# t-0hmura/pdb2reaction

Hardware: AMD Instinct MI355X
Metric: path_opt_string_iterations_per_s (higher is better)
Workload: dtype bf16x3-split

## Files before the change

pdb2reaction_amd/csrc/umx_api.hip:

```cpp
#include "umx_engine.h"
#include "umx_launch.h"
#include "umx_workspace.h"
#include "umx_periodic.h"
#include "umx_virial.h"
#include "umx_plan.h"
#include "umx_weights.h"
#include "umx_experts.h"

#define NOT_MERGED "expert-form weights are loaded but not merged: call umx_set_expert_coefficients first (then umx_set_system)"

namespace {
int energy_forces_dev_impl(umx_engine* eng, int n_images, const PosPtr d_pos, double* d_energy, float* d_forces, double* d_virial, void* hip_stream) {
  if (!eng) return UMX_ERR_ARG;
  if (eng->need_merge()) return fail(eng, UMX_ERR_ARG, "umx_energy_forces: " NOT_MERGED);
  if (!eng->have_system) return fail(eng, UMX_ERR_ARG, "umx_energy_forces: bind a system first (umx_set_system)");
  if (n_images <= 0 || !(d_pos.f || d_pos.d) || !d_energy) return fail(eng, UMX_ERR_ARG, "umx_energy_forces: bad arguments");
  if (d_virial && !d_forces) return fail(eng, UMX_ERR_ARG, "umx_energy_forces_virial: the virial comes out of the reverse pass: ask for the forces too");
  if (eng->gp_plan) return fail(eng, UMX_ERR_ARG, "umx_energy_forces: a graph-parallel evaluation is in progress (finish it with umx_gp_step)");
  CHK(periodic_check_images(eng, n_images, "umx_energy_forces"));
  HIPCHK(eng, hipSetDevice(eng->dev));
  return energy_forces_on(eng, static_cast<hipStream_t>(hip_stream), n_images, d_pos, d_energy, d_forces, d_virial);
}

template <typename P>
// ... 149 lines not shown
#ifndef UMX_SRC_DIGEST
#define UMX_SRC_DIGEST "unknown"
#endif
const char* umx_build_digest(void) { return UMX_SRC_DIGEST; }

const char* umx_last_error(const umx_engine* eng) { return eng ? eng->err.c_str() : g_create_err.c_str(); }

int umx_create(umx_engine** out, int device_ordinal) {
  if (!out) { g_create_err = "umx_create: null out pointer"; return UMX_ERR_ARG; }
  *out = nullptr;
  int n = 0;
  if (hipGetDeviceCount(&n) != hipSuccess || n <= 0) { g_create_err = "umx_create: no HIP device visible"; return UMX_ERR_NO_DEVICE; }
  if (device_ordinal < 0 || device_ordinal >= n) { g_create_err = "umx_create: device ordinal out of range"; return UMX_ERR_ARG; }
  hipDeviceProp_t prop;
  if (hipGetDeviceProperties(&prop, device_ordinal) != hipSuccess) { g_create_err = "umx_create: hipGetDeviceProperties failed"; return UMX_ERR_HIP; }
  if (std::string(prop.gcnArchName).rfind("gfx950", 0) != 0) {
    g_create_err = std::string("umx_create: device is ") + prop.gcnArchName + ", this library is built for gfx950 only";
    return UMX_ERR_NO_DEVICE;
  }
  umx_engine* e = new umx_engine();
  e->dev = device_ordinal;
  if (const char* ev = std::getenv("UMX_STREAMS")) e->n_lanes = std::atoi(ev) >= 2 ? 2 : (std::atoi(ev) == 1 ? 1 : 0);
  if (const char* ev = std::getenv("UMX_LANES_AUTO_EDGES")) e->lanes_auto_edges = std::max(0L, std::atol(ev));
  if (const char* ev = std::getenv("UMX_FORCE_PARTS")) e->force_parts = std::max(0, std::min(16, std::atoi(ev)));
  if (const char* ev = std::getenv("UMX_RECOMPUTE")) e->recompute = std::max(0, std::min(2, std::atoi(ev)));
  if (const char* ev = std::getenv("UMX_WS_GB")) e->ws_cap_default = (size_t)std::max(0L, std::atol(ev)) << 30;
  if (const char* ev = std::getenv("UMX_WS_EAGER")) e->ws_eager = std::atoi(ev) != 0;
  if (const char* ev = std::getenv("UMX_WS_SOFT_EDGES")) e->ws_soft_edges = std::max(1L, std::atol(ev));
  if (const char* ev = std::getenv("UMX_NODE_F64")) e->node_f64_on = std::atoi(ev) != 0;
  if (const char* ev = std::getenv("UMX_GRID_F64")) e->grid_f64 = std::atoi(ev) != 0;
  if (const char* ev = std::getenv("UMX_ALT_ROWS")) e->odd_sign = std::atoi(ev) != 0 ? -1.0f : 1.0f;
  if (const char* ev = std::getenv("UMX_LOW_SEP")) e->low_sep = std::atoi(ev);
  if (const char* ev = std::getenv("UMX_GEMM_HALF")) e->gemm_half = std::atoi(ev);
  if (const char* ev = std::getenv("UMX_ALIGN_PLANES")) e->align = std::atoi(ev);
  int prio_lo = 0, prio_hi = 0;
  if (hipSetDevice(device_ordinal) != hipSuccess || hipDeviceGetStreamPriorityRange(&prio_lo, &prio_hi) != hipSuccess ||
      hipStreamCreateWithFlags(&e->stream, hipStreamNonBlocking) != hipSuccess ||
      hipStreamCreateWithPriority(&e->stream2, hipStreamNonBlocking, prio_hi) != hipSuccess ||
      hipEventCreateWithFlags(&e->ev_fork, hipEventDisableTiming) != hipSuccess || hipEventCreateWithFlags(&e->ev_join, hipEventDisableTiming) != hipSuccess ||
      hipEventCreateWithFlags(&e->ev_tok[0], hipEventDisableTiming) != hipSuccess || hipEventCreateWithFlags(&e->ev_tok[1], hipEventDisableTiming) != hipSuccess ||
      hipEventCreateWithFlags(&e->ev_done, hipEventDisableTiming) != hipSuccess || hipMalloc(&e->d_flags, 4 * sizeof(int)) != hipSuccess ||
      hipMemset(e->d_flags, 0, 4 * sizeof(int)) != hipSuccess) {
    g_create_err = "umx_create: hipSetDevice/hipStreamCreate failed";
    delete e;
    return UMX_ERR_HIP;
  }
  *out = e;
  return UMX_OK;
}


int umx_destroy(umx_engine* eng) {
  if (!eng) return UMX_OK;
  gp_clear(eng);
  (void)hipSetDevice(eng->dev);
  (void)hipStreamSynchronize(eng->stream);
  for (auto& r : eng->prof) { (void)hipEventDestroy(r.a); (void)hipEventDestroy(r.b); }
  void* ptrs[] = {eng->d_w, eng->d_dw, eng->d_bw, eng->d_gmu, eng->d_z, eng->d_sysemb, eng->arena, eng->d_deg_all, eng->d_cand_all, eng->d_img_edges, eng->d_io_pos, eng->d_io_e, eng->d_io_f, eng->d_flags, eng->d_dtab, eng->d_part_deg, eng->d_part_f, eng->d_ex, eng->d_mjobs, eng->d_pjobs, eng->d_mx, eng->d_cells, eng->d_shifts_pk, eng->d_wrap, eng->d_wrap64, eng->d_lats, eng->d_io_pos64, eng->d_vir_part, eng->d_vir_wp, eng->d_io_w, eng->d_pin_src, eng->d_pin_dst, eng->d_pin_tix, eng->d_pin_wrap, eng->d_pin_deg, eng->d_pin_img, eng->d_pin_shifts};
  for (void* p : ptrs) if (p) (void)hipFree(p);
  (void)hipStreamSynchronize(eng->stream2);
  (void)hipEventDestroy(eng->ev_fork); (void)hipEventDestroy(eng->ev_join);
  (void)hipEventDestroy(eng->ev_tok[0]); (void)hipEventDestroy(eng->ev_tok[1]);
  if (eng->ev_done) (void)hipEventDestroy(eng->ev_done);
  if (eng->ev_m0) { (void)hipEventDestroy(eng->ev_m0); (void)hipEventDestroy(eng->ev_m1); }
  (void)hipStreamDestroy(eng->stream2);
  (void)hipStreamDestroy(eng->stream);
// ... 383 lines not shown
  if (!eng) return UMX_ERR_ARG;
  if (out) std::memset(out, 0, sizeof(*out));
  HIPCHK(eng, hipSetDevice(eng->dev));
  HIPCHK(eng, hipStreamSynchronize(eng->stream));
  if (eng->prof_used) HIPCHK(eng, hipEventSynchronize(eng->prof[eng->prof_used - 1].b));
  FILE* dump = nullptr;
  if (const char* dp = std::getenv("UMX_PROFILE_DUMP")) dump = std::fopen(dp, "a");
  for (size_t i = 0; i < eng->prof_used; ++i) {
    float t = 0.f;
    HIPCHK(eng, hipEventElapsedTime(&t, eng->prof[i].a, eng->prof[i].b));
    const ProfRec& r = eng->prof[i];
    if (out) {
      const int fam = r.prec > 0 ? 0 : (r.prec < 0 ? 2 : 1);
      out->ms[fam] += t; out->launches[fam] += 1; out->alg_flops[fam] += r.flops;
      out->mfma_flops[fam] += r.flops * (r.prec == 3 ? 6.0 : r.prec == 2 ? 3.0 : r.prec == 24 ? 4.0 : r.prec == 23 ? 3.0 : r.prec == 28 ? 6.0 : 1.0);
    }
    if (dump) std::fprintf(dump, "%d,%d,%d,%d,%d,%d,%d,%.6f,%.6e\n", r.M, r.N, r.K, r.amode, r.cplx, r.prec, r.gz, t, r.flops);
  }
  if (dump) std::fclose(dump);
  if (reset) eng->prof_used = 0;
  return UMX_OK;
}

int umx_debug_keep(umx_engine* eng, int on) {
  if (!eng) return UMX_ERR_ARG;
  eng->dbg_on = on != 0;
  if (!on) { eng->dbg.clear(); eng->gemm_log.clear(); }
  return UMX_OK;
}

int umx_debug_fetch(umx_engine* eng, const char* name, void* host_buf, size_t capacity, size_t* nbytes_out) {
  if (!eng || !name) return UMX_ERR_ARG;
  const std::string nm(name);
  if (nm == "gemm:table" || nm == "gemm:launches") {
    const std::string text = nm == "gemm:table" ? pl_table_text() : eng->gemm_log;
    if (nbytes_out) *nbytes_out = text.size();
    if (host_buf) {
      if (capacity < text.size()) return fail(eng, UMX_ERR_ARG, "umx_debug_fetch: buffer too small");
      std::memcpy(host_buf, text.data(), text.size());
    }
    return UMX_OK;
  }
  if (nm.rfind("weights:", 0) == 0 || nm.rfind("experts:", 0) == 0) {
    if (!eng->have_weights) return fail(eng, UMX_ERR_ARG, "umx_debug_fetch: load weights first");
    HIPCHK(eng, hipSetDevice(eng->dev));
    HIPCHK(eng, hipStreamSynchronize(eng->stream));
    const void* dptr = nullptr; size_t nb = 0;
    std::string table; float ms = 0.f;
    if (nm == "weights:w") { dptr = eng->d_w; nb = eng->n_w * sizeof(float); }
    else if (nm == "weights:dw") { dptr = eng->d_dw; nb = eng->n_dw * sizeof(float); }
    else if (nm == "weights:bw") { dptr = eng->d_bw; nb = eng->n_bw * sizeof(unsigned short); }
    else if (nm == "weights:table") {
      for (const auto& kv : eng->wt) table += kv.first + " " + std::to_string(kv.second.off) + " " + std::to_string(kv.second.count) + "\n";
      nb = table.size();
    } else if (nm == "experts:kernel_ms") {
      if (!eng->experts_merged) return fail(eng, UMX_ERR_ARG, "umx_debug_fetch: no expert merge has run");
      HIPCHK(eng, hipEventElapsedTime(&ms, eng->ev_m0, eng->ev_m1));
      nb = sizeof(float);
    } else return fail(eng, UMX_ERR_ARG, std::string("umx_debug_fetch: no buffer named ") + name);
    if (nbytes_out) *nbytes_out = nb;
    if (host_buf) {
      if (capacity < nb) return fail(eng, UMX_ERR_ARG, "umx_debug_fetch: buffer too small");
      if (dptr) HIPCHK(eng, hipMemcpy(host_buf, dptr, nb, hipMemcpyDeviceToHost));
      else if (nm == "weights:table") std::memcpy(host_buf, table.data(), nb);
      else std::memcpy(host_buf, &ms, nb);
    }
    return UMX_OK;
  }
// ... 72 lines not shown
```

pdb2reaction_amd/csrc/umx_engine.h:

```cpp
#pragma once
#include <hip/hip_runtime.h>
#include <algorithm>
#include <cmath>
#include <cstdio>
#include <cstdlib>
#include <chrono>
#include <cstring>
#include <functional>
#include <initializer_list>
#include <map>
#include <memory>
#include <set>
#include <string>
#include <type_traits>
#include <vector>

#include "../../include/umx.h"
#include "umx_common.h"
#include "umx_gemm.h"
#include "umx_gemm_pl.h"
#include "umx_gemm_q.h"
#include "umx_kernels.h"
#include "umx_edge.h"
#include "umx_graph.h"
// ... 109 lines not shown

struct Seg { bool matrix; std::function<int()> fn; float* sync_buf = nullptr; size_t sync_count = 0; };
struct Plan {
  std::vector<Seg> segs;
  void stream(std::function<int()> f) { segs.push_back({false, std::move(f)}); }
  void matrix(std::function<int()> f) { segs.push_back({true, std::move(f)}); }
  void sync(float* buf, size_t count) { Seg sg{false, nullptr}; sg.sync_buf = buf; sg.sync_count = count; segs.push_back(std::move(sg)); }
  int run_to_sync(size_t& at, const Seg** stop) {
    *stop = nullptr;
    while (at < segs.size()) {
      Seg& sg = segs[at++];
      if (sg.sync_buf) { *stop = &sg; return UMX_OK; }
      const int st = sg.fn();
      if (st != UMX_OK) return st;
    }
    return UMX_OK;
  }
};

}

struct umx_engine {
  int dev = 0;
  hipStream_t stream = nullptr;
  hipEvent_t ev_done = nullptr;
  bool ran_on_caller = false;
  int* d_flags = nullptr;
  hipStream_t stream2 = nullptr;
  hipEvent_t ev_fork = nullptr, ev_join = nullptr;
  hipEvent_t ev_tok[2] = {nullptr, nullptr};
  Precision prec;
  std::string precision;
  int low_sep = 3;
  int gemm_half = 5;
  int align = 2;
  float odd_sign = -1.0f;
  bool node_ctx = false;
  bool node_f64_on = true;
  int n_lanes = 0;
  long lanes_auto_edges = 0;
  int stream_cap = 512;
  bool throttle = false;
  bool gp = false; long gp_lo = 0, gp_hi = 0;
  std::unique_ptr<Plan> gp_plan;
  std::unique_ptr<WS> gp_ws;
  size_t gp_at = 0;
  hipStream_t gp_stream = nullptr;
  std::string err;
  bool have_weights = false;
  float* d_w = nullptr;
  float* d_dw = nullptr;
  double* d_dtab = nullptr;
  unsigned short* d_bw = nullptr;
  std::map<const float*, PlaneCopy> planes;
  std::map<std::string, Tensor> wt;
  std::vector<float> h_w;
  size_t n_w = 0, n_dw = 0, n_bw = 0;
  int n_experts = 0;
  bool experts_merged = false;
  float* d_ex = nullptr;
  MergeJob* d_mjobs = nullptr; PackJob* d_pjobs = nullptr; unsigned* d_mx = nullptr;
  int n_mjobs = 0, n_pjobs = 0, merge_blocks = 0, pack_blocks = 0;
  std::vector<const float*> f16_keys;
  hipEvent_t ev_m0 = nullptr, ev_m1 = nullptr;
  bool need_merge() const { return n_experts > 0 && !experts_merged; }
  RadialW rdeg{};
// ... 156 lines not shown
```

pdb2reaction_amd/csrc/umx_gemm_pl.h:

```cpp
#pragma once
#include "umx_gemm.h"

namespace umx {

typedef float f32x4 __attribute__((ext_vector_type(4)));

struct GemmPL {
  const unsigned short* Apl; long lda; int offA0, offA1;
  const unsigned short* Bpl; long ldb; int bHalf;
  float* Cp; long ldc; int offC, offCi;
  const float* bias;
  float conj;
  int M, N, K;
  float cscale;
  float odd_sign;
};

template <int N> __device__ __forceinline__ void wait_vmcnt() {
  asm volatile("s_waitcnt vmcnt(%0)" ::"n"(N) : "memory");
}

template <int P> __device__ __forceinline__ int pl_perm(int s, int r) {
  return P == 2 ? (s ^ ((r >> 1) & 7)) : ((s & ~3) | ((s & 3) ^ ((r >> 2) & 3)));
}

template <int JA, int JB, int TA_B, int WSTR, long TAG>
__device__ __forceinline__ void pl_issue(const GemmPL& p, unsigned char* sbase, const long (&a_off)[JA], const long (&b_off)[JB], long kofs_a, long kofs, int piece) {
#pragma unroll
  for (int j = 0; j < JA; ++j)
    __builtin_amdgcn_global_load_lds(p.Apl + a_off[j] + kofs_a, (__attribute__((address_space(3))) void*)(sbase + piece + j * WSTR), 16, 0, 0);
#pragma unroll
  for (int j = 0; j < JB; ++j)
    __builtin_amdgcn_global_load_lds(p.Bpl + b_off[j] + kofs, (__attribute__((address_space(3))) void*)(sbase + TA_B + piece + j * WSTR), 16, 0, 0);
}

template <int E> struct PlMfma;
template <> struct PlMfma<32> {
  static constexpr int NR = 16, KSTEPS = 2;
  typedef f32x16 Acc;
  static __device__ __forceinline__ int row(int lane) { return lane & 31; }
  static __device__ __forceinline__ int kc(int lane) { return lane >> 5; }
  static __device__ __forceinline__ Acc mfma(const bf16x8_t& a, const bf16x8_t& b, const Acc& c) { return __builtin_amdgcn_mfma_f32_32x32x16_bf16(a, b, c, 0, 0, 0); }
};
template <> struct PlMfma<16> {
  static constexpr int NR = 4, KSTEPS = 1;
  typedef f32x4 Acc;
  static __device__ __forceinline__ int row(int lane) { return lane & 15; }
  static __device__ __forceinline__ int kc(int lane) { return lane >> 4; }
// ... 171 lines not shown
```

pdb2reaction_amd/csrc/umx_gemm_q.h:

```cpp
#pragma once
#include <type_traits>
#include "umx_gemm_pl.h"

namespace umx {

template <int P> __device__ __forceinline__ int q_row_off(int row) { return (row >> 2) * (128 * P) + (row & 3) * (32 * P); }
template <int P> __device__ __forceinline__ int q_swz(int g) { return P == 3 ? ((g >> 2) & 1) : ((g >> 1) & 3); }
typedef _Float16 f16x8_t __attribute__((ext_vector_type(8)));

template <int JA, int JBF, int BHALF_ROUND, int A_BYTES, long TAG, int RND = 8192, class BO = long>
__device__ __forceinline__ void q3_issue(const unsigned char* A, const unsigned char* B, unsigned char* sbase, const BO (&a_off)[JA],
                                         const BO (&b_off)[JBF + BHALF_ROUND], long kofs_a, long kofs_b, int piece, bool b_tail) {
  BO ao[JA];
#pragma unroll
  for (int j = 0; j < JA; ++j) {
    ao[j] = a_off[j];
    if constexpr (sizeof(BO) == 4) asm("" : "+v"(ao[j]));
  }
#pragma unroll
  for (int j = 0; j < JA; ++j)
    __builtin_amdgcn_global_load_lds((A + kofs_a) + ao[j], (__attribute__((address_space(3))) void*)(sbase + piece + j * RND), 16, 0, 0);
  BO bo[JBF + BHALF_ROUND];
#pragma unroll
  for (int j = 0; j < JBF + BHALF_ROUND; ++j) {
    bo[j] = b_off[j];
    if constexpr (sizeof(BO) == 4) asm("" : "+v"(bo[j]));
  }
#pragma unroll
  for (int j = 0; j < JBF; ++j)
    __builtin_amdgcn_global_load_lds((B + kofs_b) + bo[j], (__attribute__((address_space(3))) void*)(sbase + A_BYTES + piece + j * RND), 16, 0, 0);
  if constexpr (BHALF_ROUND != 0)
    if (b_tail)
      __builtin_amdgcn_global_load_lds((B + kofs_b) + bo[JBF], (__attribute__((address_space(3))) void*)(sbase + A_BYTES + piece + JBF * RND), 16, 0, 0);
}

__host__ __device__ constexpr bool q_use_product(int PA, int PB, int NPROD, int qa, int qb) {
  if (PA == 3 && PB == 3) return qa + qb < 3;
  if (PA == 2 && PB == 3) return NPROD == 5 ? (qa + qb < 3) : (qa + qb < 2 || (qa == 0 && qb == 2));
  return NPROD == 4 ? true : (qa + qb < 2);
}

template <int CPLX, int WIDE, int P = 3, int S = 2, int F16 = 0, int NPROD = (P == 3 ? 6 : 3), int PB = P, int AF = 0, int LS = 0, int AL = 0, int MW = 4>
__global__ __launch_bounds__(MW * 128, MW == 4 ? 1 : 2) void umx_gemm_q_kernel(const GemmPL p) {
  static_assert(!AL || AF, "AL: the float32-A kernels");
  static_assert(!LS || (P == 3 && PB == 3 && !F16 && NPROD == 6), "LS: the six-product bf16 form");
  static_assert(LS != 2 || !WIDE, "LS = 2 (second accumulator set): 256 x 128 tiles only");
  static_assert(MW == 4 || MW == 2, "waves along M: 4 (256-row tiles) or 2 (half-height tiles, two workgroups per CU)");
  static_assert(!AF || (P == 3 && PB == 3 && F16 == 0), "AF: the six-product bf16 form with A as float32");
  static_assert((P == 3 && PB == 3 && NPROD == 6) || (P == 2 && PB == 2 && (NPROD == 3 || NPROD == 4)) || (P == 2 && PB == 3 && (NPROD == 4 || NPROD == 5)), "plane products");
  constexpr int NT = MW * 128, RND = NT * 16;
  constexpr int BM = 64 * MW, BN = WIDE ? 256 : 128;
  constexpr int BMR = CPLX ? BM / 2 : BM, BNC = CPLX ? BN / 2 : BN;
  constexpr int BLK = AF ? 256 : 128 * P, CPB = AF ? 16 : 8 * P;
  constexpr int BLKB = 128 * PB, CPBB = 8 * PB;
  constexpr int A_BYTES = AF ? BM * 64 : BM * 32 * P, B_BYTES = BN * 32 * PB, STAGE = A_BYTES + B_BYTES;
  constexpr int TNW = WIDE ? 4 : 2;
  constexpr int JA = A_BYTES / RND;
  constexpr int JBF = B_BYTES / RND, BHR = (B_BYTES % RND) ? 1 : 0;
  static_assert(S * STAGE * (MW == 4 ? 1 : 2) <= 160 * 1024 && A_BYTES % RND == 0 && (B_BYTES % RND == 0 || B_BYTES % RND == RND / 2), "tile geometry");
  static_assert((P == 2 || P == 3) && (PB == 2 || PB == 3), "two or three planes");
  static_assert(S >= 2 && S <= 4, "ring depth");
  __shared__ __attribute__((aligned(1024))) unsigned char ring[S * STAGE];
  const int tid = threadIdx.x, lane = tid & 63, wave = tid >> 6;
  const int wm = wave >> 1, wn = wave & 1;
  const int l31 = lane & 31, h = lane >> 5;

  int mt, nt;
  if (!xcd_tile<BMR, BNC>(p.M, p.N, mt, nt)) return;

  const unsigned char* Ab = reinterpret_cast<const unsigned char*>(p.Apl);
  const unsigned char* Bb = reinterpret_cast<const unsigned char*>(p.Bpl);
  const long a_blocks = p.lda / (16 * P);
  const long b_blocks = p.K / 16;
  const long gA = ((long)p.M + 3) / 4;
  const int gN = p.N / 4;
  typedef typename std::conditional<MW == 4, long, unsigned int>::type BOff;
  BOff a_off[JA], b_off[JBF + BHR];
// ... 32 lines not shown
        for (int r = 0; r < 16; ++r) low[i][j][r] = 0.f;
  }
#pragma unroll
  for (int j = 0; j < TNW; ++j) {
    float b0 = 0.f;
    if (!CPLX) {
      const int col = nt * BN + wn * (32 * TNW) + j * 32 + l31;
      b0 = (p.bias && col < p.N) ? p.bias[col] / cs : 0.f;
    }
    const float b1 = p.odd_sign < 0.f ? -b0 : b0;
#pragma unroll
    for (int i = 0; i < 2; ++i)
#pragma unroll
      for (int r = 0; r < 16; ++r) acc[i][j][r] = (r & 1) ? b1 : b0;
  }

  int a_ad[2][P], b_ad[TNW][PB];
#pragma unroll
  for (int t = 0; t < 2; ++t) {
    const int row = frag_row0<CPLX, 2, 32, BMR>(wm, t) + l31;
#pragma unroll
    for (int q = 0; q < P; ++q)
      a_ad[t][q] = AF ? ((row >> 2) * 256 + (row & 3) * 64 + ((((h * 2 + (q & 1)) ^ ((row >> 2) & 3))) * 16))
                      : (q_row_off<P>(row) + ((q * 2 + h) ^ q_swz<P>(row >> 2)) * 16);
  }
#pragma unroll
  for (int t = 0; t < TNW; ++t) {
    const int row = frag_row0<CPLX, TNW, 32, BNC>(wn, t) + l31;
#pragma unroll
    for (int q = 0; q < PB; ++q) b_ad[t][q] = A_BYTES + q_row_off<PB>(row) + ((q * 2 + h) ^ q_swz<PB>(row >> 2)) * 16;
  }

  const int nk = p.K / 16;
  constexpr long TAG = kernel_tag<CPLX, WIDE, P, S, F16, NPROD, PB, AF, LS, AL, MW>();
  constexpr int GI = JA + JBF;
#pragma unroll
  for (int t = 0; t < S - 1; ++t)
    if (t < nk) q3_issue<JA, JBF, BHR, A_BYTES, TAG, RND, BOff>(Ab + a_tile, Bb, ring + t * STAGE, a_off, b_off, (long)t * BLK, (long)t * BLKB, piece, b_tail);
  int st_cur = 0, st_nxt = S - 1;
  for (int kt = 0; kt < nk; ++kt) {
    if (S == 2 || kt + S - 2 >= nk) wait_vmcnt<0>();
    else if (BHR != 0 && b_tail) wait_vmcnt<(S - 2) * (GI + 1)>();
    else wait_vmcnt<(S - 2) * GI>();
    __builtin_amdgcn_s_barrier();
    if (kt + S - 1 < nk) q3_issue<JA, JBF, BHR, A_BYTES, TAG, RND, BOff>(Ab + a_tile, Bb, ring + st_nxt * STAGE, a_off, b_off, (long)(kt + S - 1) * BLK, (long)(kt + S - 1) * BLKB, piece, b_tail);
    const unsigned char* sb = ring + st_cur * STAGE;
    st_cur = st_cur + 1 == S ? 0 : st_cur + 1;
    st_nxt = st_nxt + 1 == S ? 0 : st_nxt + 1;
    bf16x8_t a[2][P], b[TNW][PB];
    if constexpr (AF) {
#pragma unroll
      for (int t = 0; t < 2; ++t)
        qf_split<AL>(*reinterpret_cast<const f32x4q_t*>(sb + a_ad[t][0]), *reinterpret_cast<const f32x4q_t*>(sb + a_ad[t][1]), a[t]);
    } else {
#pragma unroll
      for (int q = 0; q < P; ++q)
#pragma unroll
        for (int t = 0; t < 2; ++t) a[t][q] = *reinterpret_cast<const bf16x8_t*>(sb + a_ad[t][q]);
    }
#pragma unroll
    for (int q = 0; q < PB; ++q)
#pragma unroll
      for (int t = 0; t < TNW; ++t) b[t][q] = *reinterpret_cast<const bf16x8_t*>(sb + b_ad[t][q]);
    if constexpr (LS == 1) {
#pragma unroll
      for (int i = 0; i < 2; ++i)
#pragma unroll
// ... 16 lines not shown
          lo = __builtin_amdgcn_mfma_f32_32x32x16_f16(__builtin_bit_cast(f16x8_t, a[i][0]), __builtin_bit_cast(f16x8_t, b[j][2]), lo, 0, 0, 0);
          lo = __builtin_amdgcn_mfma_f32_32x32x16_f16(__builtin_bit_cast(f16x8_t, a[i][0]), __builtin_bit_cast(f16x8_t, b[j][1]), lo, 0, 0, 0);
          lo = __builtin_amdgcn_mfma_f32_32x32x16_f16(__builtin_bit_cast(f16x8_t, a[i][1]), __builtin_bit_cast(f16x8_t, b[j][0]), lo, 0, 0, 0);
          acc[i][j] = __builtin_amdgcn_mfma_f32_32x32x16_f16(__builtin_bit_cast(f16x8_t, a[i][0]), __builtin_bit_cast(f16x8_t, b[j][0]), acc[i][j], 0, 0, 0);
          fold_low(acc[i][j], lo);
        }
    } else
#pragma unroll
    for (int ord = P + PB - 2; ord >= 0; --ord)
#pragma unroll
      for (int qa = 0; qa < P; ++qa) {
        const int qb = ord - qa;
        if (qb < 0 || qb >= PB || !q_use_product(P, PB, NPROD, qa, qb)) continue;
#pragma unroll
        for (int i = 0; i < 2; ++i)
#pragma unroll
          for (int j = 0; j < TNW; ++j) {
            if constexpr (F16) acc[i][j] = __builtin_amdgcn_mfma_f32_32x32x16_f16(__builtin_bit_cast(f16x8_t, a[i][qa]), __builtin_bit_cast(f16x8_t, b[j][qb]), acc[i][j], 0, 0, 0);
            else if constexpr (LS == 2) {
              if (qa + qb == 2) low[i][j] = __builtin_amdgcn_mfma_f32_32x32x16_bf16(a[i][qa], b[j][qb], low[i][j], 0, 0, 0);
              else acc[i][j] = __builtin_amdgcn_mfma_f32_32x32x16_bf16(a[i][qa], b[j][qb], acc[i][j], 0, 0, 0);
            } else acc[i][j] = __builtin_amdgcn_mfma_f32_32x32x16_bf16(a[i][qa], b[j][qb], acc[i][j], 0, 0, 0);
          }
      }
  }
  if constexpr (LS == 2) {
#pragma unroll
    for (int i = 0; i < 2; ++i)
#pragma unroll
      for (int j = 0; j < TNW; ++j) fold_low(acc[i][j], low[i][j]);
  }

  const bool full = ((long)mt * BMR + BMR <= p.M) && (nt * BNC + BNC <= p.N);
  if (CPLX) {
#pragma unroll
    for (int cg = 0; cg < TNW / 2; ++cg) {
      const int chan = nt * BNC + wn * (16 * TNW) + cg * 32 + l31;
      const long e0 = (long)mt * BMR + wm * 32 + 4 * h;
      float* c = p.Cp + e0 * p.ldc + chan;
      if (full) {
#pragma unroll
        for (int r = 0; r < 16; ++r) {
          float* cr = c + (long)cd_row<16>(r) * p.ldc;
          cr[p.offC] = ((r & 1) ? cso : cs) * (acc[0][cg][r] - p.conj * acc[1][TNW / 2 + cg][r]);
          cr[p.offCi] = ((r & 1) ? cso : cs) * (acc[1][cg][r] + p.conj * acc[0][TNW / 2 + cg][r]);
        }
      } else if (chan < p.N) {
#pragma unroll
        for (int r = 0; r < 16; ++r) {
          const int dr = cd_row<16>(r);
          if (e0 + dr < p.M) {
            float* cr = c + (long)dr * p.ldc;
            cr[p.offC] = ((r & 1) ? cso : cs) * (acc[0][cg][r] - p.conj * acc[1][TNW / 2 + cg][r]);
            cr[p.offCi] = ((r & 1) ? cso : cs) * (acc[1][cg][r] + p.conj * acc[0][TNW / 2 + cg][r]);
          }
        }
      }
    }
  } else {
#pragma unroll
    for (int i = 0; i < 2; ++i)
#pragma unroll
      for (int j = 0; j < TNW; ++j) {
        const int col = nt * BN + wn * (32 * TNW) + j * 32 + l31;
        const long row0 = (long)mt * BM + wm * 64 + i * 32 + 4 * h;
        float* c = p.Cp + row0 * p.ldc + p.offC + col;
        if (full) {
// ... 15 lines not shown
```

pdb2reaction_amd/csrc/umx_launch.h:

```cpp
#pragma once

namespace {

int prof_open(umx_engine* eng, ProfRec** out, double flops, int prec, long M, int N, int K, int amode = 0, int cplx = 0, int gz = 1) {
  *out = nullptr;
  if (!eng->prof_on) return UMX_OK;
  if (eng->prof_used == eng->prof.size()) {
    ProfRec r; HIPCHK(eng, hipEventCreate(&r.a)); HIPCHK(eng, hipEventCreate(&r.b)); r.flops = 0; eng->prof.push_back(r);
  }
  ProfRec* pr = &eng->prof[eng->prof_used++];
  pr->flops = flops; pr->M = (int)M; pr->N = N; pr->K = K; pr->amode = amode; pr->cplx = cplx; pr->gz = gz; pr->prec = prec;
  HIPCHK(eng, hipEventRecord(pr->a, eng->stream));
  *out = pr;
  return UMX_OK;
}
int prof_close(umx_engine* eng, ProfRec* pr) {
  if (pr) HIPCHK(eng, hipEventRecord(pr->b, eng->stream));
  return UMX_OK;
}
inline unsigned vgrid(const umx_engine* eng, unsigned blocks) {
  return (eng->throttle && eng->stream_cap > 0 && blocks > (unsigned)eng->stream_cap) ? (unsigned)eng->stream_cap : blocks;
}

inline void launch_scan(hipStream_t s, const int* deg, long n, int* row_ptr, int* stats) {
// ... 60 lines not shown
  return launch_gemm(eng, p, R ? A_MODUL : A_PLAIN, 1);
}

int so3_linear(umx_engine* eng, const float* A, const float* Wl, const float* bias, float* Cp, long nn, const float* resid) {
  GemmP p = gp_zero();
  p.A = A; p.lda = ROW; p.offA0 = 0; p.B = Wl; p.ldb = C; p.bias = bias; p.Cp = Cp; p.ldc = ROW; p.offC = 0;
  p.M = (int)nn; p.N = C; p.K = C; p.zA = C; p.zC = C; p.resid = resid; p.ldres = ROW; p.offRes = 0; p.zRes = C; p.zBl = (long)C * C;
  NodeCtx node(eng);
  return launch_gemm(eng, p, A_PLAIN, 0, S);
}

enum PlFamily { Q_F16, Q_BF16, PL3_ROWS, PL3, PL2_WIDE, PL2_M16, PL2_M32 };

struct PlKey {
  PlFamily fam = Q_F16; bool cplx = false, wide = false, ls = false, al = false, half = false;
  bool operator==(const PlKey& o) const { return fam == o.fam && cplx == o.cplx && wide == o.wide && ls == o.ls && al == o.al && half == o.half; }
};
struct PlKernel { PlKey key; void (*fn)(const GemmPL); };

#define UMX_Q(cplx, wide, ls, al, half) \
  {{Q_BF16, cplx != 0, wide != 0, ls != 0, al != 0, half != 0}, umx_gemm_q_kernel<cplx, wide, 3, 2, 0, 6, 3, 1, (ls ? (wide ? 1 : 2) : 0), al, (half ? 2 : 4)>}
#define UMX_Q4(cplx, wide, ls) UMX_Q(cplx, wide, ls, 0, 0), UMX_Q(cplx, wide, ls, 1, 0), UMX_Q(cplx, wide, ls, 0, 1), UMX_Q(cplx, wide, ls, 1, 1)
const PlKernel pl_kernels[] = {
    {{Q_F16, false, false}, umx_gemm_q_kernel<0, 0, 2, 2, 1, 4, 3>}, {{Q_F16, true, false}, umx_gemm_q_kernel<1, 0, 2, 2, 1, 4, 3>},
    {{Q_F16, false, true}, umx_gemm_q_kernel<0, 1, 2, 2, 1, 4, 3>},  {{Q_F16, true, true}, umx_gemm_q_kernel<1, 1, 2, 2, 1, 4, 3>},
    UMX_Q4(0, 0, 0), UMX_Q4(0, 0, 1), UMX_Q4(0, 1, 0), UMX_Q4(0, 1, 1),
    UMX_Q4(1, 0, 0), UMX_Q4(1, 1, 0), UMX_Q4(1, 1, 1),
    {{PL3_ROWS}, umx_gemm_pl_kernel<16, 0, 3, 2, 4, 2, 2, 2, 1>},
    {{PL3}, umx_gemm_pl_kernel<32, 0, 3, 2, 4, 2, 2, 2>},
    {{PL2_WIDE, false, true}, umx_gemm_pl_kernel<16, 0, 2, 2, 4, 2, 2, 4>}, {{PL2_WIDE, true, true}, umx_gemm_pl_kernel<16, 1, 2, 2, 4, 2, 2, 4>},
    {{PL2_M16, false}, umx_gemm_pl_kernel<16, 0, 2, 3, 4, 2, 2, 2>},        {{PL2_M16, true}, umx_gemm_pl_kernel<16, 1, 2, 3, 4, 2, 2, 2>},
    {{PL2_M32, false}, umx_gemm_pl_kernel<32, 0, 2, 3, 4, 2, 2, 2>},
};
#undef UMX_Q
#undef UMX_Q4
std::string pl_key_text(const PlKey& k) {
  static const char* const fam[] = {"Q_F16", "Q_BF16", "PL3_ROWS", "PL3", "PL2_WIDE", "PL2_M16", "PL2_M32"};
  return std::string(fam[k.fam]) + " " + std::to_string(k.cplx) + " " + std::to_string(k.wide) + " " + std::to_string(k.ls) + " " + std::to_string(k.al) + " " +
         std::to_string(k.half);
}
std::string pl_table_text() {
  std::string t;
  for (const PlKernel& e : pl_kernels) t += pl_key_text(e.key) + "\n";
  return t;
}

struct PlChoice { PlKey key; unsigned blocks = 0; long lda = 0, ldb = 0; int prec = 0; const char* err = nullptr; };
PlChoice choose_pl(const Precision& pm, Pass pass, bool w_quad, int cplx, long M, int N, int K, int a_cols, bool a_f32rows, int low_sep, int align, int half) {
  PlChoice c;
  c.key.cplx = cplx != 0;
  const bool fwd = pass == FWD;
  const int P = fwd ? 3 : pm.rev_planes;
  c.prec = (fwd && pm.fwd_fmt == 1) ? 24 : P;
  c.lda = (long)a_cols * P; c.ldb = (long)K * P;
  const int bmr = cplx ? 128 : 256;
  const long nM = (M + bmr - 1) / bmr;
  const bool fills = nM * (N / (cplx ? 128 : 256)) >= 256;
  c.key.ls = fwd && pm.fwd_fmt == 3 && (low_sep == 2 || (low_sep == 3 && !cplx) || (low_sep == 1 && !cplx && K == RH));
  c.key.wide = N % (cplx ? 128 : 256) == 0 && (fills || c.key.ls);
  int bnc = c.key.wide ? (cplx ? 128 : 256) : (cplx ? 64 : 128);
  if (fwd && pm.fwd_fmt == 1) {
    c.key.fam = Q_F16; c.lda = (long)a_cols * 2; c.ldb = (long)K * 3;
  } else if (fwd || (P == 3 && w_quad)) {
    c.key.fam = Q_BF16; c.lda = (long)a_cols * 3; c.ldb = (long)K * 3;
    c.key.al = fwd && (align == 1 || (align == 2 && !cplx));
  } else if (P == 3) {
    if (cplx || N > 128) { c.err = "gemm_pl: three-plane PL products are instantiated for the plain N <= 128 (radial fc3^T) products only"; return c; }
    c.key.fam = a_f32rows ? PL3_ROWS : PL3;
    if (a_f32rows) c.lda = (long)a_cols * 2;
  } else if (c.key.wide) {
    c.key.fam = PL2_WIDE;
  } else {
    c.key.fam = (cplx || K >= 512) ? PL2_M16 : PL2_M32;
  }
  c.key.half = c.key.fam == Q_BF16 && (half == 3 || (half == 4 && cplx) || (half == 5 && !c.key.ls && K >= 256) ||
                               (fwd && c.key.ls && (half == 2 || (half == 1 && !c.key.wide))));
  const long nMf = c.key.half ? (M + bmr / 2 - 1) / (bmr / 2) : nM;
  c.blocks = (unsigned)(((nMf + 7) / 8) * 8 * ((N + bnc - 1) / bnc));
  return c;
}

int gemm_pl(umx_engine* eng, int cplx, Pass pass, const unsigned short* Apl, int a_cols, int offA0, int offA1, const float* Wkey, int bHalf,
            const float* bias, float* Cp, long ldc, int offC, int offCi, long M, int N, int K, float conj, bool a_f32rows = false) {
  if (M <= 0) return UMX_OK;
  auto it = eng->planes.find(Wkey);
  if (it == eng->planes.end()) return fail(eng, UMX_ERR_ARG, "gemm_pl: weight has no PL copy");
  if (K % 32 != 0) return fail(eng, UMX_ERR_ARG, "gemm_pl: K not a multiple of 32");
  const PlaneCopy& w = it->second;
  const PlChoice c = choose_pl(eng->prec, pass, w.quad, cplx, M, N, K, a_cols, a_f32rows, eng->low_sep, eng->align, eng->gemm_half);
  if (c.err) return fail(eng, UMX_ERR_ARG, c.err);
  const PlKernel* k = nullptr;
  for (const PlKernel& e : pl_kernels)
    if (e.key == c.key) { k = &e; break; }
  if (!k) return fail(eng, UMX_ERR_ARG, "gemm_pl: variant not instantiated");
  GemmPL q;
  std::memset(&q, 0, sizeof(q));
  q.Apl = Apl; q.lda = c.lda; q.offA0 = offA0; q.offA1 = offA1; q.Bpl = w.ptr; q.ldb = c.ldb; q.bHalf = bHalf;
  q.Cp = Cp; q.ldc = ldc; q.offC = offC; q.offCi = offCi; q.bias = bias; q.conj = conj; q.M = (int)M; q.N = N; q.K = K;
  q.odd_sign = eng->odd_sign;
  if (c.key.fam == Q_F16) q.cscale = 1.0f / (QF16_SCALE * w.scale);
  ProfRec* pr;
  CHK(prof_open(eng, &pr, cplx ? 8.0 * M * (double)N * K : 2.0 * M * (double)N * K, c.prec, M, N, K, 9, cplx));
  hipLaunchKernelGGL(k->fn, dim3(c.blocks), dim3(c.key.half ? 256 : 512), 0, eng->stream, q);
  HIPCHK(eng, hipGetLastError());
  if (eng->dbg_on)
    eng->gemm_log += std::string(pass == FWD ? "fwd " : "rev ") + pl_key_text(c.key) + " " + std::to_string(M) + " " + std::to_string(N) + " " + std::to_string(K) + " " +
                     std::to_string(c.blocks) + "\n";
  return prof_close(eng, pr);
}

struct So2Layout { int ld, m0, m1re, m1im, m1w, m2re, m2im, m2w; };
constexpr So2Layout SO2_Y1 = {XROT, 768, 768, 1280, 512, 1792, 2048, 256};
constexpr So2Layout SO2_HG = {HG, 640, 640, 896, 256, 1152, 1280, 128};
constexpr So2Layout SO2_MSG = {ROW, 384, 384, 640, 256, 896, 1024, 128};
constexpr int SO2_RAD_M1 = 768, SO2_RAD_M2 = 1280;

int so2_conv(umx_engine* eng, Pass pass, const void* A, const So2Layout& la, float* Cp, const So2Layout& lc, const float* Wm0, const float* Wm1,
             const float* Wm2, const float* bias, long ne, float conj, const float* R = nullptr) {
  if (eng->prec.planes) {
    const unsigned short* Apl = static_cast<const unsigned short*>(A);
    CHK(gemm_pl(eng, 0, pass, Apl, la.ld, 0, 0, Wm0, 0, bias, Cp, lc.ld, 0, 0, ne, lc.m0, la.m0, 1.0f));
    CHK(gemm_pl(eng, 1, pass, Apl, la.ld, la.m1re, la.m1im, Wm1, lc.m1w, nullptr, Cp, lc.ld, lc.m1re, lc.m1im, ne, lc.m1w, la.m1w, conj));
    return gemm_pl(eng, 1, pass, Apl, la.ld, la.m2re, la.m2im, Wm2, lc.m2w, nullptr, Cp, lc.ld, lc.m2re, lc.m2im, ne, lc.m2w, la.m2w, conj);
  }
  const float* Af = static_cast<const float*>(A);
  GemmP p = gp_zero();
  p.A = Af; p.lda = la.ld; p.R = R; p.ldr = R ? RAD : 0; p.B = Wm0; p.ldb = la.m0; p.bias = bias;
  p.Cp = Cp; p.ldc = lc.ld; p.M = (int)ne; p.N = lc.m0; p.K = la.m0;
  CHK(launch_gemm(eng, p, R ? A_MODUL : A_PLAIN, 0));
  CHK(gemm_cplx(eng, Af, la.ld, la.m1re, la.m1im, R, R ? RAD : 0, R ? SO2_RAD_M1 : 0, Wm1, la.m1w, lc.m1w, Cp, lc.ld, lc.m1re, lc.m1im, ne, lc.m1w, la.m1w, conj));
  return gemm_cplx(eng, Af, la.ld, la.m2re, la.m2im, R, R ? RAD : 0, R ? SO2_RAD_M2 : 0, Wm2, la.m2w, lc.m2w, Cp, lc.ld, lc.m2re, lc.m2im, ne, lc.m2w, la.m2w, conj);
}

}
```

pdb2reaction_amd/csrc/umx_plan.h:

```cpp
#pragma once

namespace {

enum OpFmt {
  OP_QUAD,
  OP_HALVES,
  OP_PLANES,
  OP_ROWS
};
OpFmt fwd_operand(const Precision& p) { return !p.planes ? OP_ROWS : p.fwd_fmt == 1 ? OP_HALVES : OP_QUAD; }
OpFmt rev_operand(const Precision& p) { return p.rev_quad() ? OP_QUAD : OP_PLANES; }
std::string link_tag(int slot) { return slot == NL ? ".deg" : "." + std::to_string(slot); }
int dbg_operand(umx_engine* eng, const char* base, int slot, OpFmt fmt, const void* ptr, long ne, long cols, int planes = 2) {
  if (!eng->dbg_on) return UMX_OK;
  const long rows = (fmt == OP_QUAD || fmt == OP_HALVES) ? (ne + 3) / 4 * 4 : ne;
  const size_t elem = fmt == OP_PLANES ? 2 * (size_t)planes : 4;
  return dbg_capture(eng, std::string(base) + (fmt == OP_QUAD ? "q" : fmt == OP_HALVES ? "h" : fmt == OP_PLANES ? "pl" : "") + link_tag(slot), ptr, (size_t)rows * cols * elem);
}

#define UMX_LAUNCH(kernel, grid, ...) hipLaunchKernelGGL(kernel, dim3(grid), dim3(256), 0, eng->stream, __VA_ARGS__)

int link_radial_head(umx_engine* eng, const WS& w, const RadialW& r, int slot, long ne) {
  const bool planes = eng->prec.planes && eng->planes.count(r.w3);
  const unsigned tiles = nblk(ne, 64);
// ... 332 lines not shown
  UMX_LAUNCH(k_grid_expand, nblk(nn, 4), w.G0, eng->from_grid, G, w.gridA, nn);
  if (eng->dbg_on) DBG("g_gridout" + t, w.gridA, ng * C);
  CHK(gemm_grid(eng, w.gridA, C, 0, L.g3T, C, nullptr, w.gridB, H, 0, ng, H, C));
  if (eng->dbg_on) DBG("g_gsil2" + t, w.gridB, ng * H);
  UMX_LAUNCH(k_silu_bwd, nblk(ng * H, 256), w.gridB, (long)H, w.ffg2[i], w.gridA, ng, H);
  if (eng->dbg_on) DBG("g_ffg2" + t, w.gridA, ng * H);
  CHK(gemm_grid(eng, w.gridA, H, 0, L.g2T, H, nullptr, w.gridB, H, 0, ng, H, H));
  if (eng->dbg_on) DBG("g_gsil1" + t, w.gridB, ng * H);
  UMX_LAUNCH(k_silu_bwd, nblk(ng * H, 256), w.gridB, (long)H, w.ffg1[i], w.gridA, ng, H);
  if (eng->dbg_on) DBG("g_ffg1" + t, w.gridA, ng * H);
  CHK(gemm_grid(eng, w.gridA, H, 0, L.g1T, H, nullptr, w.gridB, C, 0, ng, C, H));
  if (eng->dbg_on) DBG("g_gridin" + t, w.gridB, ng * C);
  UMX_LAUNCH(k_grid_contract, nblk(nn, 4), w.gridB, eng->to_grid, G, (const float*)nullptr, w.G1, nn);
  if (eng->dbg_on) DBG("g_xn2" + t, w.G1, nn * ROW);
  return UMX_OK;
}

void plan_atomwise_bwd(Plan& P, WS& w, const ChunkCtx& c, int i) {
  P.stream([c, &w, i]() -> int {
    UMX_STAGE(c);
    CHK(eng->ff_grid ? atomwise_bwd_grid(c, w, i) : atomwise_bwd_spectral(c, w, i));
    UMX_LAUNCH(k_norm_bwd, nblk(nn, 4), w.G1, w.xs[2 * i + 1], eng->lw[i].n2w, w.G0, w.G2, nn);
    HIPCHK(eng, hipGetLastError());
    DBG("g_xmid." + std::to_string(i), w.G2, nn * ROW);
    if (ne > 0 && eng->prec.planes) CHK(link_rotate_back_bwd(eng, w, i, ne));
    return UMX_OK;
  });
}

void plan_edge_bwd(Plan& P, WS& w, const ChunkCtx& c, int i) {
  if (c.ne <= 0) return;
  const LayerW* L = &c.eng->lw[i];
  if (c.eng->prec.planes) {
    P.matrix([=, &w]() -> int { return so2_conv(c.eng, REV, w.gmsgpl, SO2_MSG, w.hid, SO2_MSG, L->c2m0T, L->c2m1T, L->c2m2T, nullptr, c.ne, -1.0f); });
    P.stream([=, &w]() -> int {
      UMX_STAGE(c);
      DBG("g_hid." + std::to_string(i), w.hid, ne * ROW);
      return link_gate_bwd(eng, w, i, ne);
    });
    P.matrix([=, &w]() -> int { return so2_conv(c.eng, REV, w.ghgpl, SO2_HG, w.gy1, SO2_Y1, L->c1m0T, L->c1m1T, L->c1m2T, nullptr, c.ne, -1.0f); });
    P.matrix([=, &w]() -> int {
      UMX_STAGE(c);
      DBG("g_y1." + std::to_string(i), w.gy1, ne * XROT);
      return link_modrot_bwd(eng, w, i, nn, ne);
    });
    P.matrix([=, &w]() -> int { return radial_bwd_fc3(c.eng, w, L->rad, c.ne, nullptr, w.gradpl, c.eng->prec.rev_quad()); });
    P.stream([=, &w]() -> int { return radial_bwd_tail(c.eng, w, L->rad, i, c.ne); });
    return;
  }
  P.stream([=, &w]() -> int {
    UMX_STAGE(c);
    const std::string t = "." + std::to_string(i);
    CHK(link_rotate_back_bwd(eng, w, i, ne));
    CHK(so2_conv(eng, REV, w.gmsg, SO2_MSG, w.hid, SO2_MSG, L->c2m0T, L->c2m1T, L->c2m2T, nullptr, ne, -1.0f));
    DBG("g_msg" + t, w.gmsg, ne * ROW); DBG("g_hid" + t, w.hid, ne * ROW);
    CHK(link_gate_bwd(eng, w, i, ne));
    CHK(so2_conv(eng, REV, w.ghg, SO2_HG, w.gy1, SO2_Y1, L->c1m0T, L->c1m1T, L->c1m2T, nullptr, ne, -1.0f));
    DBG("g_hg" + t, w.ghg, ne * HG); DBG("g_y1" + t, w.gy1, ne * XROT);
    if (c.fused_rev) CHK(link_modrot_bwd(eng, w, i, nn, ne));
    else {
      CHK(link_gather_rotate(eng, w, i, ne));
      UMX_LAUNCH(k_modulate_bwd, nblk(ne, 4), w.gy1, w.xrot, w.rad[i], w.grad, w.tau, ne);
      DBG("g_xrot" + t, w.gy1, ne * XROT); DBG("g_rad" + t, w.grad, ne * RAD);
    }
    return radial_bwd(eng, w, L->rad, i, ne, w.grad);
  });
}

void plan_norm1_bwd(Plan& P, WS& w, const ChunkCtx& c, int i) {
  const bool have_gxn = c.ne > 0 && c.fused_rev;
  auto gather_rotate_bwd = [c, &w]() -> int {
    UMX_STAGE(c);
// ... 537 lines not shown
```

Baseline: 1.949.

## Fuse gate-reverse elementwise step into reverse SO(2) GEMM epilogue

Measured after the change: 1.979 (median of 6 runs). +1.6%, better.

```diff
diff --git a/pdb2reaction_amd/csrc/umx_api.hip b/pdb2reaction_amd/csrc/umx_api.hip
--- a/pdb2reaction_amd/csrc/umx_api.hip
+++ b/pdb2reaction_amd/csrc/umx_api.hip
@@ -205,6 +205,7 @@
   if (const char* ev = std::getenv("UMX_ALT_ROWS")) e->odd_sign = std::atoi(ev) != 0 ? -1.0f : 1.0f;
   if (const char* ev = std::getenv("UMX_LOW_SEP")) e->low_sep = std::atoi(ev);
   if (const char* ev = std::getenv("UMX_GEMM_HALF")) e->gemm_half = std::atoi(ev);
+  if (const char* ev = std::getenv("UMX_GATE_EPI")) e->gate_epi = std::max(0, std::min(2, std::atoi(ev)));
   if (const char* ev = std::getenv("UMX_ALIGN_PLANES")) e->align = std::atoi(ev);
   int prio_lo = 0, prio_hi = 0;
   if (hipSetDevice(device_ordinal) != hipSuccess || hipDeviceGetStreamPriorityRange(&prio_lo, &prio_hi) != hipSuccess ||
@@ -654,8 +655,8 @@
 int umx_debug_fetch(umx_engine* eng, const char* name, void* host_buf, size_t capacity, size_t* nbytes_out) {
   if (!eng || !name) return UMX_ERR_ARG;
   const std::string nm(name);
-  if (nm == "gemm:table" || nm == "gemm:launches") {
-    const std::string text = nm == "gemm:table" ? pl_table_text() : eng->gemm_log;
+  if (nm == "gemm:table" || nm == "gemm:table_gate" || nm == "gemm:launches") {
+    const std::string text = nm == "gemm:table" ? pl_table_text() : nm == "gemm:table_gate" ? pl_gate_table_text() : eng->gemm_log;
     if (nbytes_out) *nbytes_out = text.size();
     if (host_buf) {
       if (capacity < text.size()) return fail(eng, UMX_ERR_ARG, "umx_debug_fetch: buffer too small");
diff --git a/pdb2reaction_amd/csrc/umx_engine.h b/pdb2reaction_amd/csrc/umx_engine.h
--- a/pdb2reaction_amd/csrc/umx_engine.h
+++ b/pdb2reaction_amd/csrc/umx_engine.h
@@ -165,6 +165,7 @@
   Precision prec;
   std::string precision;
   int low_sep = 3;
+  int gate_epi = 1;
   int gemm_half = 5;
   int align = 2;
   float odd_sign = -1.0f;
diff --git a/pdb2reaction_amd/csrc/umx_gemm_pl.h b/pdb2reaction_amd/csrc/umx_gemm_pl.h
--- a/pdb2reaction_amd/csrc/umx_gemm_pl.h
+++ b/pdb2reaction_amd/csrc/umx_gemm_pl.h
@@ -14,6 +14,7 @@
   int M, N, K;
   float cscale;
   float odd_sign;
+  const float* hg; float* ghg; float* gate_acc; int ep_mode;
 };
 
 template <int N> __device__ __forceinline__ void wait_vmcnt() {
diff --git a/pdb2reaction_amd/csrc/umx_gemm_q.h b/pdb2reaction_amd/csrc/umx_gemm_q.h
--- a/pdb2reaction_amd/csrc/umx_gemm_q.h
+++ b/pdb2reaction_amd/csrc/umx_gemm_q.h
@@ -40,9 +40,59 @@
   return NPROD == 4 ? true : (qa + qb < 2);
 }
 
-template <int CPLX, int WIDE, int P = 3, int S = 2, int F16 = 0, int NPROD = (P == 3 ? 6 : 3), int PB = P, int AF = 0, int LS = 0, int AL = 0, int MW = 4>
+__device__ __forceinline__ long qf_index(long row, int cols, int k) { return ((row >> 2) * (cols >> 4) + (k >> 4)) * 64 + (row & 3) * 16 + (k & 15); }
+template <int MODE, bool FULL, class G>
+__device__ __forceinline__ void gate_epilogue(const GemmPL& p, long e0, int col, G g) {
+  constexpr int NV = MODE == 0 ? 1 : 2;
+  const int c = col & (H - 1), blk = col >> 7;
+  const int deg = MODE == 0 ? blk - 1 : MODE == 1 ? blk : 1;
+  const int row_o[2] = {MODE == 0 ? blk : MODE == 1 ? 3 + blk : 7, MODE == 0 ? blk : MODE == 1 ? 5 + blk : 8};
+  const bool finish = (MODE == 1 && deg == 0) || MODE == 2;
+  const long M4 = ((long)p.M + 3) & ~3L;
+  float gate[2][4], hp[2][NV][4], a[2][4];
+  auto request = [&](int b, int q4) {
+#pragma unroll
+    for (int q = 0; q < 4; ++q) {
+      const long e = e0 + 8 * q4 + q;
+      const float* hr = p.hg + (FULL || e < p.M ? e : (long)p.M - 1) * HG;
+      gate[b][q] = deg >= 0 ? hr[deg * H + c] : 0.f;
+#pragma unroll
+      for (int v = 0; v < NV; ++v) hp[b][v][q] = hr[2 * H + row_o[v] * H + c];
+      a[b][q] = (MODE != 0 && (FULL || e < p.M)) ? p.gate_acc[e * (2 * H) + deg * H + c] : 0.f;
+    }
+  };
+  request(0, 0);
+#pragma unroll
+  for (int q4 = 0; q4 < 4; ++q4) {
+    const int b = q4 & 1;
+    if (q4 < 3) request(b ^ 1, q4 + 1);
+#pragma unroll
+    for (int q = 0; q < 4; ++q) {
+      const int r = 4 * q4 + q;
+      const long e = e0 + 8 * q4 + q;
+      const bool in = FULL || e < p.M;
+      if (!FULL && e >= M4) continue;
+      const float rs = (q & 1) ? p.odd_sign : 1.0f;
+      float s = 0.f, acc = a[b][q];
+      if (deg >= 0) s = sigmoid_f(gate[b][q]);
+#pragma unroll
+      for (int v = 0; v < NV; ++v) {
+        const float gv = g(v, r);
+        const float w = deg < 0 ? gv * silu_grad_f(hp[b][v][q]) : gv * s;
+        p.ghg[qf_index(e, HG, 2 * H + row_o[v] * H + c)] = in ? rs * w : 0.f;
+        if (deg >= 0) acc = __builtin_fmaf(gv, hp[b][v][q], acc);
+      }
+      if (deg < 0) continue;
+      if (finish) p.ghg[qf_index(e, HG, deg * H + c)] = in ? rs * (acc * s * (1.0f - s)) : 0.f;
+      else if (in) p.gate_acc[e * (2 * H) + deg * H + c] = acc;
+    }
+  }
+}
+
+template <int CPLX, int WIDE, int P = 3, int S = 2, int F16 = 0, int NPROD = (P == 3 ? 6 : 3), int PB = P, int AF = 0, int LS = 0, int AL = 0, int MW = 4, int EP = 0>
 __global__ __launch_bounds__(MW * 128, MW == 4 ? 1 : 2) void umx_gemm_q_kernel(const GemmPL p) {
   static_assert(!AL || AF, "AL: the float32-A kernels");
+  static_assert(!EP || (AF && !LS && !AL && (CPLX || !WIDE)), "EP (gate-reverse epilogue): the six-product float32-A form; plain narrow, complex narrow or wide");
   static_assert(!LS || (P == 3 && PB == 3 && !F16 && NPROD == 6), "LS: the six-product bf16 form");
   static_assert(LS != 2 || !WIDE, "LS = 2 (second accumulator set): 256 x 128 tiles only");
   static_assert(MW == 4 || MW == 2, "waves along M: 4 (256-row tiles) or 2 (half-height tiles, two workgroups per CU)");
@@ -141,7 +191,7 @@
   }
 
   const int nk = p.K / 16;
-  constexpr long TAG = kernel_tag<CPLX, WIDE, P, S, F16, NPROD, PB, AF, LS, AL, MW>();
+  constexpr long TAG = kernel_tag<CPLX, WIDE, P, S, F16, NPROD, PB, AF, LS, AL, MW, EP>();
   constexpr int GI = JA + JBF;
 #pragma unroll
   for (int t = 0; t < S - 1; ++t)
@@ -224,7 +274,35 @@
   }
 
   const bool full = ((long)mt * BMR + BMR <= p.M) && (nt * BNC + BNC <= p.N);
-  if (CPLX) {
+  if constexpr (EP != 0) {
+    if constexpr (CPLX) {
+      auto column = [&](auto cg_) {
+        constexpr int cg = decltype(cg_)::value;
+        int chan = nt * BNC + wn * (16 * TNW) + cg * 32 + l31;
+        long e0 = (long)mt * BMR + wm * 32 + 4 * h;
+        asm volatile("" : "+v"(chan), "+v"(e0));
+        auto g = [&](int v, int r) -> float {
+          return v == 0 ? ((r & 1) ? cso : cs) * __builtin_fmaf(-p.conj, acc[1][TNW / 2 + cg][r], acc[0][cg][r])
+                        : ((r & 1) ? cso : cs) * __builtin_fmaf(p.conj, acc[0][TNW / 2 + cg][r], acc[1][cg][r]);
+        };
+        if (p.ep_mode == 2) { if (full) gate_epilogue<2, true>(p, e0, chan, g); else if (chan < p.N) gate_epilogue<2, false>(p, e0, chan, g); }
+        else                { if (full) gate_epilogue<1, true>(p, e0, chan, g); else if (chan < p.N) gate_epilogue<1, false>(p, e0, chan, g); }
+      };
+      column(std::integral_constant<int, 0>());
+      if constexpr (TNW / 2 > 1) column(std::integral_constant<int, 1>());
+    } else {
+#pragma unroll
+      for (int i = 0; i < 2; ++i)
+#pragma unroll
+        for (int j = 0; j < TNW; ++j) {
+          int col = nt * BN + wn * (32 * TNW) + j * 32 + l31;
+          long row0 = (long)mt * BM + wm * 64 + i * 32 + 4 * h;
+          asm volatile("" : "+v"(col), "+v"(row0));
+          auto g = [&](int, int r) -> float { return ((r & 1) ? cso : cs) * acc[i][j][r]; };
+          if (full) gate_epilogue<0, true>(p, row0, col, g); else if (col < p.N) gate_epilogue<0, false>(p, row0, col, g);
+        }
+    }
+  } else if (CPLX) {
 #pragma unroll
     for (int cg = 0; cg < TNW / 2; ++cg) {
       const int chan = nt * BNC + wn * (16 * TNW) + cg * 32 + l31;
diff --git a/pdb2reaction_amd/csrc/umx_launch.h b/pdb2reaction_amd/csrc/umx_launch.h
--- a/pdb2reaction_amd/csrc/umx_launch.h
+++ b/pdb2reaction_amd/csrc/umx_launch.h
@@ -116,16 +116,25 @@
     {{PL2_M16, false}, umx_gemm_pl_kernel<16, 0, 2, 3, 4, 2, 2, 2>},        {{PL2_M16, true}, umx_gemm_pl_kernel<16, 1, 2, 3, 4, 2, 2, 2>},
     {{PL2_M32, false}, umx_gemm_pl_kernel<32, 0, 2, 3, 4, 2, 2, 2>},
 };
+struct GateEpi { const float* hg; float* ghg; float* acc; int mode; };
+#define UMX_QG(cplx, wide, half) {{Q_BF16, cplx != 0, wide != 0, false, false, half != 0}, umx_gemm_q_kernel<cplx, wide, 3, 2, 0, 6, 3, 1, 0, 0, (half ? 2 : 4), 1>}
+const PlKernel pl_gate_kernels[] = {UMX_QG(0, 0, 0), UMX_QG(0, 0, 1), UMX_QG(1, 0, 0), UMX_QG(1, 0, 1), UMX_QG(1, 1, 0), UMX_QG(1, 1, 1)};
+#undef UMX_QG
 #undef UMX_Q
 #undef UMX_Q4
-std::string pl_key_text(const PlKey& k) {
+std::string pl_key_text(const PlKey& k, bool gate = false) {
   static const char* const fam[] = {"Q_F16", "Q_BF16", "PL3_ROWS", "PL3", "PL2_WIDE", "PL2_M16", "PL2_M32"};
-  return std::string(fam[k.fam]) + " " + std::to_string(k.cplx) + " " + std::to_string(k.wide) + " " + std::to_string(k.ls) + " " + std::to_string(k.al) + " " +
+  return std::string(fam[k.fam]) + (gate ? "_GATE " : " ") + std::to_string(k.cplx) + " " + std::to_string(k.wide) + " " + std::to_string(k.ls) + " " + std::to_string(k.al) + " " +
          std::to_string(k.half);
 }
 std::string pl_table_text() {
   std::string t;
   for (const PlKernel& e : pl_kernels) t += pl_key_text(e.key) + "\n";
+  return t;
+}
+std::string pl_gate_table_text() {
+  std::string t;
+  for (const PlKernel& e : pl_gate_kernels) t += pl_key_text(e.key, true) + "\n";
   return t;
 }
 
@@ -165,7 +174,8 @@
 }
 
 int gemm_pl(umx_engine* eng, int cplx, Pass pass, const unsigned short* Apl, int a_cols, int offA0, int offA1, const float* Wkey, int bHalf,
-            const float* bias, float* Cp, long ldc, int offC, int offCi, long M, int N, int K, float conj, bool a_f32rows = false) {
+            const float* bias, float* Cp, long ldc, int offC, int offCi, long M, int N, int K, float conj, bool a_f32rows = false,
+            const GateEpi* gate = nullptr) {
   if (M <= 0) return UMX_OK;
   auto it = eng->planes.find(Wkey);
   if (it == eng->planes.end()) return fail(eng, UMX_ERR_ARG, "gemm_pl: weight has no PL copy");
@@ -174,7 +184,9 @@
   const PlChoice c = choose_pl(eng->prec, pass, w.quad, cplx, M, N, K, a_cols, a_f32rows, eng->low_sep, eng->align, eng->gemm_half);
   if (c.err) return fail(eng, UMX_ERR_ARG, c.err);
   const PlKernel* k = nullptr;
-  for (const PlKernel& e : pl_kernels)
+  if (gate && (c.key.fam != Q_BF16 || pass != REV || N % 128 != 0)) return fail(eng, UMX_ERR_ARG, "gemm_pl: the gate-reverse epilogue goes with the reverse Q_BF16 products");
+  if (gate) { for (const PlKernel& e : pl_gate_kernels) if (e.key == c.key) { k = &e; break; } }
+  else for (const PlKernel& e : pl_kernels)
     if (e.key == c.key) { k = &e; break; }
   if (!k) return fail(eng, UMX_ERR_ARG, "gemm_pl: variant not instantiated");
   GemmPL q;
@@ -182,13 +194,14 @@
   q.Apl = Apl; q.lda = c.lda; q.offA0 = offA0; q.offA1 = offA1; q.Bpl = w.ptr; q.ldb = c.ldb; q.bHalf = bHalf;
   q.Cp = Cp; q.ldc = ldc; q.offC = offC; q.offCi = offCi; q.bias = bias; q.conj = conj; q.M = (int)M; q.N = N; q.K = K;
   q.odd_sign = eng->odd_sign;
+  if (gate) { q.hg = gate->hg; q.ghg = gate->ghg; q.gate_acc = gate->acc; q.ep_mode = gate->mode; }
   if (c.key.fam == Q_F16) q.cscale = 1.0f / (QF16_SCALE * w.scale);
   ProfRec* pr;
   CHK(prof_open(eng, &pr, cplx ? 8.0 * M * (double)N * K : 2.0 * M * (double)N * K, c.prec, M, N, K, 9, cplx));
   hipLaunchKernelGGL(k->fn, dim3(c.blocks), dim3(c.key.half ? 256 : 512), 0, eng->stream, q);
   HIPCHK(eng, hipGetLastError());
   if (eng->dbg_on)
-    eng->gemm_log += std::string(pass == FWD ? "fwd " : "rev ") + pl_key_text(c.key) + " " + std::to_string(M) + " " + std::to_string(N) + " " + std::to_string(K) + " " +
+    eng->gemm_log += std::string(pass == FWD ? "fwd " : "rev ") + pl_key_text(c.key, gate != nullptr) + " " + std::to_string(M) + " " + std::to_string(N) + " " + std::to_string(K) + " " +
                      std::to_string(c.blocks) + "\n";
   return prof_close(eng, pr);
 }
@@ -200,12 +213,14 @@
 constexpr int SO2_RAD_M1 = 768, SO2_RAD_M2 = 1280;
 
 int so2_conv(umx_engine* eng, Pass pass, const void* A, const So2Layout& la, float* Cp, const So2Layout& lc, const float* Wm0, const float* Wm1,
-             const float* Wm2, const float* bias, long ne, float conj, const float* R = nullptr) {
+             const float* Wm2, const float* bias, long ne, float conj, const float* R = nullptr, const GateEpi* gate = nullptr) {
   if (eng->prec.planes) {
     const unsigned short* Apl = static_cast<const unsigned short*>(A);
-    CHK(gemm_pl(eng, 0, pass, Apl, la.ld, 0, 0, Wm0, 0, bias, Cp, lc.ld, 0, 0, ne, lc.m0, la.m0, 1.0f));
-    CHK(gemm_pl(eng, 1, pass, Apl, la.ld, la.m1re, la.m1im, Wm1, lc.m1w, nullptr, Cp, lc.ld, lc.m1re, lc.m1im, ne, lc.m1w, la.m1w, conj));
-    return gemm_pl(eng, 1, pass, Apl, la.ld, la.m2re, la.m2im, Wm2, lc.m2w, nullptr, Cp, lc.ld, lc.m2re, lc.m2im, ne, lc.m2w, la.m2w, conj);
+    GateEpi g[3];
+    for (int m = 0; m < 3 && gate; ++m) { g[m] = *gate; g[m].mode = m; }
+    CHK(gemm_pl(eng, 0, pass, Apl, la.ld, 0, 0, Wm0, 0, bias, Cp, lc.ld, 0, 0, ne, lc.m0, la.m0, 1.0f, false, gate ? &g[0] : nullptr));
+    CHK(gemm_pl(eng, 1, pass, Apl, la.ld, la.m1re, la.m1im, Wm1, lc.m1w, nullptr, Cp, lc.ld, lc.m1re, lc.m1im, ne, lc.m1w, la.m1w, conj, false, gate ? &g[1] : nullptr));
+    return gemm_pl(eng, 1, pass, Apl, la.ld, la.m2re, la.m2im, Wm2, lc.m2w, nullptr, Cp, lc.ld, lc.m2re, lc.m2im, ne, lc.m2w, la.m2w, conj, false, gate ? &g[2] : nullptr);
   }
   const float* Af = static_cast<const float*>(A);
   GemmP p = gp_zero();
diff --git a/pdb2reaction_amd/csrc/umx_plan.h b/pdb2reaction_amd/csrc/umx_plan.h
--- a/pdb2reaction_amd/csrc/umx_plan.h
+++ b/pdb2reaction_amd/csrc/umx_plan.h
@@ -388,12 +388,23 @@
   if (c.ne <= 0) return;
   const LayerW* L = &c.eng->lw[i];
   if (c.eng->prec.planes) {
-    P.matrix([=, &w]() -> int { return so2_conv(c.eng, REV, w.gmsgpl, SO2_MSG, w.hid, SO2_MSG, L->c2m0T, L->c2m1T, L->c2m2T, nullptr, c.ne, -1.0f); });
-    P.stream([=, &w]() -> int {
-      UMX_STAGE(c);
-      DBG("g_hid." + std::to_string(i), w.hid, ne * ROW);
-      return link_gate_bwd(eng, w, i, ne);
-    });
+    const int ge = c.eng->gate_epi;
+    const bool fills = (c.ne + 127) / 128 * (SO2_MSG.m1w / 128) >= 256;
+    if (c.eng->prec.rev_quad() && (ge == 2 || (ge == 1 && !c.eng->dbg_on && fills))) {
+      P.matrix([=, &w]() -> int {
+        UMX_STAGE(c);
+        const GateEpi gate{w.hg[i], reinterpret_cast<float*>(w.ghgpl), w.hid, 0};
+        CHK(so2_conv(eng, REV, w.gmsgpl, SO2_MSG, w.hid, SO2_MSG, L->c2m0T, L->c2m1T, L->c2m2T, nullptr, ne, -1.0f, nullptr, &gate));
+        return dbg_operand(eng, "ghg", i, OP_QUAD, w.ghgpl, ne, HG);
+      });
+    } else {
+      P.matrix([=, &w]() -> int { return so2_conv(c.eng, REV, w.gmsgpl, SO2_MSG, w.hid, SO2_MSG, L->c2m0T, L->c2m1T, L->c2m2T, nullptr, c.ne, -1.0f); });
+      P.stream([=, &w]() -> int {
+        UMX_STAGE(c);
+        DBG("g_hid." + std::to_string(i), w.hid, ne * ROW);
+        return link_gate_bwd(eng, w, i, ne);
+      });
+    }
     P.matrix([=, &w]() -> int { return so2_conv(c.eng, REV, w.ghgpl, SO2_HG, w.gy1, SO2_Y1, L->c1m0T, L->c1m1T, L->c1m2T, nullptr, c.ne, -1.0f); });
     P.matrix([=, &w]() -> int {
       UMX_STAGE(c);
```
